# sjpark0905/DNA-LDPC-codes

Hardware: AMD Instinct MI355X
Metric: decoded codewords/sec (n=18432, m=2048, 50 BP iters) at 1/2/4/8 GPUs; % HBM roofline (higher is better)
Workload: dtype f64; 1 GPU; bsc-p0.02-100k-per-gpu-bp50; code=decode_n18432_m2048_final.pchk (8,72)-regular, E=147456, input=int8 channel codes in HBM + table code*ln49 (LR = host exp), batch_per_gpu=100000, global_batch=100000, max_iter=50, algo=bp, parallelism=dp1 (contiguous codeword shards, no collective), resident_per_pass=192, group_tiles=3, nontemporal_d=False, continuous=True, resident_pool=True, syndrome_split=False

## Files before the change

dna-ldpc-codes_amd/csrc/engine.hip:

```cpp
#include <hip/hip_ext.h>
#include <hip/hip_runtime.h>

#include <algorithm>
#include <cmath>
#include <cstdio>
#include <cstdlib>
#include <cstring>
#include <thread>

#include "engine.hpp"
#include "kernels.hpp"
#include "kernels_int.hpp"
#include "encode_kernels.hpp"

namespace ldpc {

constexpr int32_t kDefaultGroupTiles = 3;
constexpr int32_t kDefaultMsaGroupTiles = 8;
constexpr int32_t kDefaultVarCpw = 4;
constexpr int32_t kDefaultVarCpwCoded = 2;
constexpr int32_t kDefaultPoolTiles = 3;
constexpr int32_t kDefaultResPoll = 8;
constexpr int32_t kDefaultSynBlocks = 32;
constexpr int64_t kMsaPool = 1024;
constexpr int64_t kResAutoMaxTiles = 4;
constexpr int kProbes = 4;

constexpr int32_t kDefaultFlags = LDPC_SCHED_NONTEMPORAL | LDPC_SCHED_CONTINUOUS | LDPC_SCHED_MSA_COMPRESSED |
                                  LDPC_SCHED_RESIDENT | LDPC_SCHED_FIRST_FROM_PRIOR | LDPC_SCHED_LR_TABLE;
constexpr int32_t kAllFlags = kDefaultFlags | LDPC_SCHED_DEBUG_NO_DRAIN | LDPC_SCHED_DEBUG_BAD_LANE;

constexpr int32_t kResolved = 1 << 30, kResChosen = 1 << 29;

ldpc_schedule resolve_schedule(const ldpc_schedule* s)
{
    ldpc_schedule r{};
    if (s) r = *s;
    r.flags_set &= kAllFlags;
    r.flags = (kDefaultFlags & ~r.flags_set) | (r.flags & r.flags_set);
    r.flags &= kAllFlags;
    r.flags_set = kAllFlags | kResolved | ((r.flags_set & LDPC_SCHED_RESIDENT) ? kResChosen : 0);
    if (r.group_tiles == 0) r.group_tiles = -2;
    if (r.var_cpw < 1 || r.var_cpw > 8 || (r.var_cpw > 4 && r.var_cpw != 8)) r.var_cpw = -2;
    if (r.pool_tiles <= 0) r.pool_tiles = 0;
// ... 29 lines not shown
    return 2 * g.E * 8 + (int64_t)g.N * 8 + (g.N + 7) / 8 + 8;
}

Engine::~Engine()
{
    if (device >= 0) hipSetDevice(device);
    if (stream) hipStreamSynchronize(stream);
    for (int c = 0; c < K_NCLASS; c++)
        for (auto& p : ev_live[c]) { hipEventDestroy(p.first); hipEventDestroy(p.second); }
    for (auto e : ev_pool) hipEventDestroy(e);
    hipFree(d_fresh); hipFree(d_occ); hipFree(d_lane_b); hipFree(d_lane_n); hipFree(d_ctr);
    if (h_poll) hipHostFree(h_poll);
    if (h_fault) hipHostFree(h_fault);
    hipFree(d_row_ptr); hipFree(d_col_idx); hipFree(d_col_idx_T); hipFree(d_col_ptr); hipFree(d_col_edge); hipFree(d_col_er); hipFree(d_row_pos);
    hipFree(d_unsat); hipFree(d_done); hipFree(d_fin); hipFree(d_fin_b); hipFree(d_fin_n);
    hipFree(d_sgn);
    hipFree(v2c); if (c2v != v2c) hipFree(c2v); hipFree(prior); hipFree(hard); hipFree(active); hipFree(iters); hipFree(valid);
    hipFree(post_t);
    hipFree(pcode); hipFree(d_ptab); hipFree(d_expand);
    if (h_ptab) hipHostFree(h_ptab);
    if (stream) hipStreamDestroy(stream);
}

template <typename T>
static int upload(T** dst, const std::vector<T>& v)
{
    const size_t n = std::max<size_t>(v.size(), 1);
    LDPC_HIP(hipMalloc((void**)dst, n * sizeof(T)));
    if (!v.empty()) LDPC_HIP(hipMemcpy(*dst, v.data(), v.size() * sizeof(T), hipMemcpyHostToDevice));
    return LDPC_OK;
// ... 49 lines not shown

    const bool reg_72_8 = g->regular_dc && g->dc_max == 72 && g->regular_dv && g->dv_max == 8;
    msa_c = algo == LDPC_ALGO_MSA && reg_72_8 && g->N % 16 == 0 && g->E < ((int64_t)1 << dev::MSA_ER_SHIFT) &&
            sched_flag(sched, LDPC_SCHED_MSA_COMPRESSED);
    cont = sched_flag(sched, LDPC_SCHED_CONTINUOUS) && !int_algo &&
           (reg_72_8 || (g->regular_dv && g->dv_max == 8) || gen_bucket(g->dv_max, kGenVarBuckets) != 0);
    const bool gen_res = !reg_72_8 && gen_bucket(g->dc_max, kGenCheckBuckets) != 0 &&
                         gen_bucket(g->dv_max, kGenVarBuckets) != 0;
    res = sched_flag(sched, LDPC_SCHED_RESIDENT) && cont && !msa_c && ((reg_72_8 && g->N % 32 == 0) || gen_res);
    const bool res_chosen = (sched.flags_set & kResChosen) != 0;
    if (res && !res_chosen && chunk > kResAutoMaxTiles * 64) res = false;
    if (res && !res_chosen && reg_72_8 && sched.pool_tiles <= 0 &&
        64.0 * 8.0 * kDefaultPoolTiles * ((double)g->E + (double)g->N) > 1.15 * kGenPoolBytes)
        res = false;
    nt_d = sched_flag(sched, LDPC_SCHED_NONTEMPORAL) && !res;
    debug_no_drain = sched_flag(sched, LDPC_SCHED_DEBUG_NO_DRAIN);
    debug_bad_lane = sched_flag(sched, LDPC_SCHED_DEBUG_BAD_LANE);
    var_cpw = sched.var_cpw;
    res_poll = sched.poll_every;
    if (chunk <= 0) {
        size_t fr = 0, tot = 0;
        LDPC_HIP(hipMemGetInfo(&fr, &tot));
        const int64_t ptiles = sched.pool_tiles > 0 ? sched.pool_tiles : reg_72_8 ? kDefaultPoolTiles : gen_pool_tiles(*g);
        const int64_t want = res ? 64 * ptiles : (msa_c && cont) ? kMsaPool : 16384;
        chunk = std::min<int64_t>(want, (int64_t)(fr / 2) / engine_bytes_per_codeword(*g));
    }
    cap = std::max<int64_t>(64, (chunk + 63) / 64 * 64);
    cap_tiles = cap / 64;
    if (cap_tiles > 65535) { set_error("chunk too large (max 4194240 codewords)"); return LDPC_ERR_ARG; }
    int64_t group = sched.group_tiles;
// ... 35 lines not shown
        LDPC_HIP(hipMalloc((void**)&d_lane_n, (size_t)cap * sizeof(int32_t)));
        LDPC_HIP(hipMalloc((void**)&d_ctr, (size_t)(1 + kRing) * sizeof(unsigned long long)));
        LDPC_HIP(hipHostMalloc((void**)&h_poll, (size_t)kRing * sizeof(unsigned long long),
                               hipHostMallocCoherent | hipHostMallocMapped));
        std::memset(h_poll, 0, (size_t)kRing * sizeof(unsigned long long));
        LDPC_HIP(hipHostGetDevicePointer((void**)&d_poll, h_poll, 0));
        LDPC_HIP(hipHostMalloc((void**)&h_fault, dev::kFaultWords * sizeof(unsigned long long),
                               hipHostMallocCoherent | hipHostMallocMapped));
        std::memset(h_fault, 0, dev::kFaultWords * sizeof(unsigned long long));
        LDPC_HIP(hipHostGetDevicePointer((void**)&d_fault, h_fault, 0));
        LDPC_HIP(hipMalloc((void**)&d_unsat, (size_t)cap_tiles * sizeof(unsigned long long)));
        LDPC_HIP(hipMalloc((void**)&d_done, (size_t)cap_tiles * sizeof(unsigned int)));
        LDPC_HIP(hipMalloc((void**)&d_fin, (size_t)cap_tiles * sizeof(uint64_t)));
        LDPC_HIP(hipMalloc((void**)&d_fin_b, (size_t)cap * sizeof(int64_t)));
        LDPC_HIP(hipMalloc((void**)&d_fin_n, (size_t)cap * sizeof(int32_t)));
        syn_blocks = res ? 0 : sched.syn_blocks;
        first_fp = !res && reg_72_8 && algo == LDPC_ALGO_BP && sched_flag(sched, LDPC_SCHED_FIRST_FROM_PRIOR);
    }
    const size_t E = (size_t)std::max<int64_t>(g->E, 1);
    LDPC_HIP(hipMalloc((void**)&v2c, (size_t)cap * E * sizeof(double)));
    if (res) {
        c2v_tiles = cap_tiles;
        c2v = v2c;
    } else {
        c2v_tiles = std::max<int64_t>(group_tiles, cont ? (cap_tiles + 3) / 4 : 0);
        c2v_bytes = msa_c ? msa_scratch_bytes(c2v_tiles, g->M) : (size_t)c2v_tiles * 64 * E * sizeof(double);
        LDPC_HIP(hipMalloc((void**)&c2v, c2v_bytes));
    }
    LDPC_HIP(hipMalloc((void**)&prior, (size_t)cap * g->N * sizeof(double)));
    if (msa_c) LDPC_HIP(hipMalloc((void**)&d_sgn, (size_t)cap * g->N));
    LDPC_HIP(hipMalloc((void**)&hard, (size_t)cap_tiles * g->N * sizeof(uint64_t)));
    LDPC_HIP(hipMalloc((void**)&active, (size_t)cap_tiles * sizeof(uint64_t)));
    LDPC_HIP(hipMalloc((void**)&iters, (size_t)cap * sizeof(int32_t)));
    LDPC_HIP(hipMalloc((void**)&valid, (size_t)cap * sizeof(uint8_t)));
    if (!int_algo && (res || group_tiles < cap_tiles)) return probe(kProbes);
    return LDPC_OK;
}

int32_t Engine::flags() const
{
    return (nt_d ? LDPC_SCHED_NONTEMPORAL : 0) | (cont ? LDPC_SCHED_CONTINUOUS : 0) |
           (msa_c ? LDPC_SCHED_MSA_COMPRESSED : 0) | (res ? LDPC_SCHED_RESIDENT : 0) |
           (syn_blocks > 0 ? LDPC_SCHED_SPLIT_SYNDROME : 0) | (first_fp ? LDPC_SCHED_FIRST_FROM_PRIOR : 0) |
           (sched.flags & (LDPC_SCHED_LR_TABLE | LDPC_SCHED_DEBUG_NO_DRAIN | LDPC_SCHED_DEBUG_BAD_LANE));
}

int Engine::probe(int probes)
{
    const size_t E = (size_t)std::max<int64_t>(g->E, 1);
    const size_t bytes = res ? (size_t)cap * E * sizeof(double) : c2v_bytes;
    const unsigned gt = (unsigned)(res ? cap_tiles : std::min<int64_t>(group_tiles, cap_tiles));
    LDPC_HIP(hipMemsetAsync(v2c, 0, (size_t)gt * 64 * E * sizeof(double), stream));
    LDPC_HIP(hipMemsetAsync(prior, 0, (size_t)gt * 64 * g->N * sizeof(double), stream));
    LDPC_HIP(hipMemsetAsync(active, 0xff, (size_t)gt * sizeof(uint64_t), stream));
    if (d_sgn) LDPC_HIP(hipMemsetAsync(d_sgn, 0, (size_t)gt * 64 * g->N, stream));
    std::vector<double*> cand{res ? v2c : c2v};
    for (int i = 1; i < probes; i++) {
        double* p = nullptr;
// ... 632 lines not shown

int Engine::run_cont_steps(const double* d_in, int in_kind, int64_t B, int32_t max_iter, uint8_t* d_hard,
                           double* d_post, int post_kind, int32_t* d_iters, uint8_t* d_valid)
{
    using namespace dev;
    const int msa = algo == LDPC_ALGO_MSA;
    if (msa && in_kind == LDPC_IN_LR) { set_error("min-sum takes LLR input"); return LDPC_ERR_ARG; }
    if (msa && post_kind == LDPC_POST_RATIO) { set_error("LDPC_POST_RATIO is BP-only"); return LDPC_ERR_ARG; }
    if (!d_hard || !d_iters || !d_valid) { set_error("continuous mode needs hard, iters and valid outputs"); return LDPC_ERR_ARG; }
    const int32_t M = g->M, N = g->N;
    const int64_t tiles = std::min<int64_t>(cap_tiles, (B + 63) / 64);
    if (d_post && !post_t) LDPC_HIP(hipMalloc((void**)&post_t, (size_t)cap * N * sizeof(double)));
    double* pt = d_post ? post_t : nullptr;
    static_assert(1 + kRing <= 256, "occupancy ring");
    LAUNCH(K_OTHER, klaunch(k_cont_reset, dim3((unsigned)std::min<int64_t>((tiles + 255) / 256, 1024)), dim3(256), 0,
                            stream, active, d_fresh, d_occ, d_ctr, 1 + kRing, d_unsat, d_done, tiles));
    ContState cs{active, d_fresh, d_occ, d_lane_b, d_lane_n, d_ctr, nullptr, B};
    cs.ntiles = tiles;
    cs.fault = d_fault;
    cs.debug_bad_lane = debug_bad_lane ? 1 : 0;
    const uint64_t q0 = poll_seq;
    ResStep rs{hard, d_col_idx, d_unsat, d_done, d_fin, d_fin_b, d_fin_n, N, max_iter, cs, ContOut{d_iters, d_valid},
               d_row_ptr};
    const bool syn72 = g->regular_dc && g->dc_max == 72;
    const int hard_vec = ((uintptr_t)d_hard % 8 == 0 && N % 8 == 0) ? 1 : 0;
    Refill rf{d_fresh, d_lane_b, d_in, in_kind == LDPC_IN_LLR ? 1 : 0, d_fin, d_fin_b, d_fin_n,
              d_hard, d_post, post_kind == LDPC_POST_RATIO ? 1 : 0, hard_vec};
    rf.nb = B;
    rf.fault = d_fault;
    if (cur_codes) {
        rf.in = nullptr;
        rf.in_code = cur_codes;
        rf.pcode = pcode;
        rf.ptab = d_ptab;
    }
    const bool single_fill = B <= tiles * 64;
    const int lag = single_fill ? 1 : kLag;
    const int64_t lanes = tiles * 64;
    const int64_t windows = (B + lanes - 1) / lanes + 1;
    auto step_limit = [&](int64_t every) {
        return windows * ((int64_t)max_iter + 2) + (int64_t)(lag + 2) * every + 8;
    };
    auto drained = [&](unsigned long long occ) { return occ == 0 && !debug_no_drain; };
    auto overrun = [&](int64_t steps) {
// ... 165 lines not shown
```

dna-ldpc-codes_amd/csrc/engine.hpp:

```cpp
#pragma once
#include <hip/hip_runtime.h>

#include <cstdint>
#include <memory>
#include <mutex>
#include <string>
#include <vector>

#include "../../include/ldpc_amd.h"
#include "graph.hpp"
#include "kargs.hpp"

namespace ldpc {

void set_error(const std::string& msg);
const char* last_error();

#define LDPC_HIP(call)                                                                           \
    do {                                                                                         \
        hipError_t _e = (call);                                                                  \
        if (_e != hipSuccess) {                                                                  \
            ::ldpc::set_error(std::string(#call) + ": " + hipGetErrorString(_e));                \
            return LDPC_ERR_DEVICE;                                                              \
        }                                                                                        \
// ... 8 lines not shown
    const HostGraph* g = nullptr;
    int device = 0;
    int algo = LDPC_ALGO_BP;
    hipStream_t stream = nullptr;
    ldpc_schedule sched{};
    int64_t cap = 0;
    int64_t cap_tiles = 0;
    int64_t group_tiles = 0;
    int64_t c2v_tiles = 0;
    size_t c2v_bytes = 0;
    bool nt_d = false;
    bool cont = false;
    bool msa_c = false;
    bool res = false;
    bool first_fp = false;
    bool debug_no_drain = false;
    bool debug_bad_lane = false;
    int var_cpw = 4;
    int res_poll = 8;
    int syn_blocks = 0;
    uint8_t* d_sgn = nullptr;
    unsigned long long* d_unsat = nullptr;
    unsigned int* d_done = nullptr;
    uint64_t* d_fin = nullptr;
    int64_t* d_fin_b = nullptr;
    int32_t* d_fin_n = nullptr;
    const dev::ResStep* rstep = nullptr;
    static constexpr int kRing = 8, kLag = 2;
    uint64_t* d_fresh = nullptr;
    uint64_t* d_occ = nullptr;
    int64_t* d_lane_b = nullptr;
    int32_t* d_lane_n = nullptr;
    unsigned long long* d_ctr = nullptr;
    uint64_t poll_seq = 0;
    unsigned long long* h_poll = nullptr;
    unsigned long long* d_poll = nullptr;
    void poll_arm(dev::ContState& cs, uint64_t q) const;
    int poll_wait(uint64_t q, unsigned long long* occ);
    unsigned long long* h_fault = nullptr;
    unsigned long long* d_fault = nullptr;
    int check_fault();
// ... 89 lines not shown
```

dna-ldpc-codes_amd/csrc/kargs.hpp:

```cpp
#pragma once
#include <cstdint>

namespace ldpc {
namespace dev {

struct Refill {
    const uint64_t* fresh;
    const int64_t* lane_b;
    const double* in;
    int in_is_llr;
    const uint64_t* fin;
    const int64_t* fin_b;
    const int32_t* fin_n;
    uint8_t* hard_out;
    double* post_out;
    int post_ratio;
    int hard_vec;
    int prior_only = 0;
    const int8_t* in_code = nullptr;
    int8_t* pcode = nullptr;
    const double* ptab = nullptr;
    int64_t nb = 0;
    unsigned long long* fault = nullptr;
};

constexpr unsigned long long kFaultTag = 1ull << 63;
constexpr unsigned long long kFaultIndex = (1ull << 48) - 1ull;
enum FaultKind : unsigned {
    kFaultIters = 1,
    kFaultOutput = 2,
    kFaultRefill = 3,
    kFaultSchedule = 4
};
constexpr int kFaultWords = 5;

constexpr int kCodeBias = 128;

struct ContState {
// ... 20 lines not shown
    uint8_t* valid;
};

struct ResStep {
    const uint64_t* hard;
    const int32_t* col_idx;
    unsigned long long* unsat;
    unsigned int* done;
    uint64_t* fin;
    int64_t* fin_b;
    int32_t* fin_n;
    int32_t N, max_iter;
    ContState cs;
    ContOut co;
    const int32_t* row_ptr = nullptr;
};

}
}
```

dna-ldpc-codes_amd/csrc/kernels.hpp:

```cpp
#pragma once
#include <hip/hip_runtime.h>
#include <cstdint>

#include "kargs.hpp"

namespace ldpc {
namespace dev {

constexpr int TILE = 64;

__device__ __forceinline__ int wave_id() { return __builtin_amdgcn_readfirstlane((int)(threadIdx.x >> 6)); }
__device__ __forceinline__ int lane_id() { return (int)(threadIdx.x & 63); }

__device__ __forceinline__ unsigned xcd_block(unsigned b, unsigned nb)
{
    const unsigned q = nb / 8, r = nb % 8, x = b % 8;
    return (x < r ? x * (q + 1) : r * (q + 1) + (x - r) * q) + b / 8;
}

__device__ __forceinline__ uint64_t shfl_xor_u64(uint64_t v, int m)
{
    uint32_t lo = (uint32_t)v, hi = (uint32_t)(v >> 32);
    lo = (uint32_t)__shfl_xor((int)lo, m);
    hi = (uint32_t)__shfl_xor((int)hi, m);
// ... 68 lines not shown
#pragma unroll
        for (int c = 0; c < CPW; ++c) p[c] = (uint8_t)(v >> (8 * c));
    }
}

__host__ __device__ __forceinline__ uint64_t splitmix64(uint64_t x)
{
    x += 0x9E3779B97F4A7C15ull;
    x = (x ^ (x >> 30)) * 0xBF58476D1CE4E5B9ull;
    x = (x ^ (x >> 27)) * 0x94D049BB133111EBull;
    return x ^ (x >> 31);
}

__device__ __forceinline__ void cont_lanes(int64_t t, uint64_t occ, uint64_t U, int32_t max_iter, const ContState& cs,
                                           const ContOut& co, int64_t* s_b, int32_t* s_n, uint64_t* s_fin,
                                           int32_t ln0, int64_t b0, bool probe)
{
    const int lane = lane_id();
    {
        const size_t li = (size_t)t * TILE + lane;
        const bool o = (occ >> lane) & 1ull;
        const int32_t ln = o ? ln0 : 0;
        const bool unsat = (U >> lane) & 1ull;
        const bool fin = o && (!unsat || ln == max_iter);
        const bool cont = o && !fin;
        const int64_t b = o ? b0 : -1;
        if (fin && lane_index_ok(b, cs.B, cs.fault, kFaultIters)) { co.iters[b] = ln; co.valid[b] = unsat ? 0 : 1; }
        s_b[lane] = b;
        s_n[lane] = ln;
        const uint64_t F = __ballot(fin), Cm = __ballot(cont);
        const uint64_t freem = ~Cm;
        const int nfree = __popcll(freem);
        unsigned long long base = 0;
        if (lane == 0 && nfree > 0) {
            if (probe) {
                const unsigned long long nb = __hip_atomic_load(cs.next_b, __ATOMIC_RELAXED, __HIP_MEMORY_SCOPE_AGENT);
                base = (nb < (unsigned long long)cs.B) ? atomicAdd(cs.next_b, (unsigned long long)nfree) : nb;
            } else {
                base = atomicAdd(cs.next_b, (unsigned long long)nfree);
            }
        }
        base = __shfl(base, 0);
        const int rank = __popcll(freem & ((1ull << lane) - 1ull));
        const bool fresh = !cont && (base + (unsigned long long)rank < (unsigned long long)cs.B);
        const uint64_t Fr = __ballot(fresh);
        if (cont) cs.lane_n[li] = ln + 1;
        if (fresh) {
            int64_t nbv = (int64_t)(base + rank);
            if (cs.debug_bad_lane && nbv == 0) nbv = cs.B + 4096;
            cs.lane_b[li] = nbv;
            cs.lane_n[li] = 0;
        }
        if (lane == 0) {
            cs.active[t] = Cm;
            cs.fresh[t] = Fr;
            cs.occupied[t] = Cm | Fr;
            *s_fin = F;
            if (cs.occ_count) {
                const unsigned long long add = (1ull << kOccTileShift) | (unsigned long long)__popcll(Cm | Fr);
                const unsigned long long old = atomicAdd(cs.occ_count, add);
                if (cs.poll_host && (int64_t)(old >> kOccTileShift) + 1 == cs.ntiles)
                    __hip_atomic_store(cs.poll_host, (cs.poll_tag << kOccTileShift) | ((old + add) & kOccMask),
                                       __ATOMIC_RELAXED, __HIP_MEMORY_SCOPE_SYSTEM);
            }
            if (t == 0 && cs.occ_clear) *cs.occ_clear = 0ull;
        }
    }
}

template <int DC>
__device__ __forceinline__ uint64_t row_parity(const uint64_t* __restrict__ h, const int32_t* __restrict__ cols)
{
    const int lane = lane_id();
    uint64_t p = 0;
#pragma unroll
    for (int k0 = 0; k0 < DC; k0 += TILE)
        if (k0 + lane < DC) p ^= h[cols[k0 + lane]];
#pragma unroll
    for (int off = 32; off > 0; off >>= 1) p ^= shfl_xor_u64(p, off);
    return p;
}

__device__ __forceinline__ void res_arrive(int64_t t, uint64_t occ, uint64_t p, const ResStep& rs, int32_t ln0,
                                           int64_t b0, uint32_t nblk)
{
    __shared__ uint64_t red[4];
    __shared__ int64_t s_b[TILE];
    __shared__ int32_t s_n[TILE];
    __shared__ uint64_t s_fin;
    __shared__ int s_last;
    const int lane = lane_id(), w = wave_id();
    if (lane == 0) red[w] = p;
    __syncthreads();
    if (threadIdx.x == 0) {
        const uint64_t U = red[0] | red[1] | red[2] | red[3];
        unsigned long long o = 0;
        if (U) o = atomicOr(rs.unsat + t, (unsigned long long)U);
        asm volatile("" ::"v"(o) : "memory");
        s_last = atomicAdd(rs.done + t, 1u) == nblk - 1;
    }
    __syncthreads();
    if (!s_last) return;
    if (threadIdx.x < TILE) {
        const uint64_t U = occ ? (uint64_t)atomicOr(rs.unsat + t, 0ull) : 0ull;
        cont_lanes(t, occ, U, rs.max_iter, rs.cs, rs.co, s_b, s_n, &s_fin, ln0, b0, false);
        const size_t li = (size_t)t * TILE + lane;
        rs.fin_b[li] = s_b[lane];
        rs.fin_n[li] = s_n[lane];
        if (lane == 0) {
            rs.fin[t] = s_fin;
            atomicExch(rs.unsat + t, 0ull);
            atomicExch(rs.done + t, 0u);
        }
    }
}

__global__ __launch_bounds__(256) void k_init(const double* __restrict__ in, int in_is_llr, int algo_msa,
                                              int64_t Bc, int32_t N, int64_t E,
                                              const int32_t* __restrict__ col_ptr, const int32_t* __restrict__ col_edge,
                                              double* __restrict__ prior, double* __restrict__ v2c,
                                              uint64_t* __restrict__ hard, uint64_t* __restrict__ active,
                                              int32_t* __restrict__ iters, uint8_t* __restrict__ valid,
                                              uint8_t* __restrict__ sgn, int32_t vpa, int32_t vpb)
{
    __shared__ double s[TILE][TILE + 1];
    const int lane = lane_id(), w = wave_id();
// ... 130 lines not shown
    const int lane = lane_id();
    const int32_t row = (int32_t)rb * 4 + wave_id();
    const uint64_t act = RES ? rs.cs.occupied[t] : active[t];
    const auto src = dmsg + ((size_t)t * E + (size_t)row * DC) * TILE + lane;
    const auto dst = lr_t + (size_t)row * DC * TILE + lane;
    if constexpr (!RES) {
        if (!(row < M && line_occupied(act, lane))) return;
        double x[DC];
        check_bp_load<DC, NT, false>(x, src);
        check_bp_compute<DC, false>(x, dst);
    } else {
        static_assert(DC <= 2 * TILE, "row parity: two gathers per lane");
        const bool occ_l = (act >> lane) & 1ull;
        const int32_t ln0 = rs.cs.lane_n[t * TILE + lane];
        const int64_t b0 = rs.cs.lane_b[t * TILE + lane];
        uint64_t par = 0;
        if (row < M && act != 0) {
            const int32_t* __restrict__ cols = rs.col_idx + (size_t)row * DC;
            const int32_t c0 = cols[lane < DC ? lane : DC - 1];
            const int32_t c1 = cols[TILE + lane < DC ? TILE + lane : DC - 1];
            double x[DC];
            check_bp_load<DC, NT, true>(x, src);
            int32_t d0 = c0, d1 = c1;
            asm volatile("" : "+v"(d0), "+v"(d1));
            const uint64_t* __restrict__ h = rs.hard + (size_t)t * rs.N;
            const uint64_t g0 = h[d0];
            const uint64_t g1 = h[d1];
            check_bp_compute<DC, true>(x, dst);
            uint64_t p = (lane < DC ? g0 : 0ull) ^ (TILE + lane < DC ? g1 : 0ull);
#pragma unroll
            for (int off = 32; off > 0; off >>= 1) p ^= shfl_xor_u64(p, off);
            par = p;
        }
        res_arrive(t, act, par, rs, occ_l ? ln0 : 0, occ_l ? b0 : 0, nrb);
    }
}

template <int DC, bool PC = false>
__global__ __launch_bounds__(256, 2) void k_check_bp_first(const double* __restrict__ prior,
                                                           const int8_t* __restrict__ pcode,
                                                           const double* __restrict__ ptab,
                                                           const int32_t* __restrict__ col_idx,
                                                           double* __restrict__ lr, const uint64_t* __restrict__ active,
                                                           int32_t M, int32_t N, int64_t E, int64_t t0)
{
    const int lane = lane_id();
    const int32_t row = (int32_t)blockIdx.x * 4 + wave_id();
    const int64_t t = t0 + blockIdx.y;
    const uint64_t act = active[t];
// ... 101 lines not shown

template <bool MSA, int DV, bool NT, bool CONT, int CPW, bool INPLACE, bool PC = false>
__device__ __forceinline__ void var_m_block(typename Msg<INPLACE>::in c2v_t, typename Msg<INPLACE>::out v2c,
                                            double* __restrict__ prior, uint64_t* __restrict__ hard,
                                            const uint64_t* __restrict__ active, const int32_t* __restrict__ col_edge,
                                            double* __restrict__ post, int32_t N, int64_t E, int64_t t, uint32_t cb,
                                            const Refill& rf)
{
    const int lane = lane_id();
    const int32_t j0 = ((int32_t)cb * 4 + wave_id()) * CPW;
    if (j0 >= N) return;
    const uint64_t act = active[t];
    const uint64_t frm = CONT ? rf.fresh[t] : 0ull;
    const uint64_t touched = act | frm;
    const uint64_t fm = (CONT && rf.fin) ? rf.fin[t] : 0ull;
    if (touched == 0 && fm == 0) return;
    const bool live = (act >> lane) & 1ull;
    const bool fr = CONT && ((frm >> lane) & 1ull);
    const bool fl = (fm >> lane) & 1ull;
    int64_t fb = 0;
    int32_t fn = 0;
    if (fl) {
        fb = rf.fin_b[t * TILE + lane];
        fn = rf.fin_n[t * TILE + lane];
    }
    const size_t tb = (size_t)t * E;
    int32_t eid[CPW][DV];
#pragma unroll
    for (int c = 0; c < CPW; ++c)
#pragma unroll
        for (int s = 0; s < DV; ++s) eid[c][s] = col_edge[(size_t)(j0 + c) * DV + s];
    double l[CPW][DV], pv[CPW], xin[CPW];
    int8_t kin[CPW];
    bool bad_in = false;
// ... 8 lines not shown
        }
    }
    if (live) {
#pragma unroll
        for (int c = 0; c < CPW; ++c) {
            pv[c] = prior_at<PC>(prior, rf, ((size_t)t * N + j0 + c) * TILE + lane);
#pragma unroll
            for (int s = 0; s < DV; ++s) l[c][s] = c2v_t[(size_t)eid[c][s] * TILE + lane];
        }
    }
    if constexpr (PC) {
        if (fr) {
#pragma unroll
            for (int c = 0; c < CPW; ++c) xin[c] = rf.ptab[kin[c] + kCodeBias];
        }
    }
    const bool fok = out_ok(fb, rf);
    if (CONT && fl && fok) {
        uint64_t hw[CPW];
#pragma unroll
        for (int c = 0; c < CPW; ++c) hw[c] = hard[(size_t)t * N + j0 + c];
        store_fin_hard<CPW>(rf, hw, fb, N, j0, lane);
    }
#pragma unroll
    for (int c = 0; c < CPW; ++c) {
        const int32_t j = j0 + c;
        const size_t pj = ((size_t)t * N + j) * TILE + lane;
        if (CONT && fl && fok && rf.post_out) {
            const size_t ob = (size_t)fb * N + j;
            const double pv = fn > 0 ? post[pj] : prior_at<PC>(prior, rf, pj);
// ... 12 lines not shown
        if (fr) {
            const double x = xin[c];
            if (MSA) {
                np = x;
#pragma unroll
                for (int s = 0; s < DV; ++s) dv[s] = x;
                h = !(x > 0);
            } else {
                const double LR0 = (!PC && rf.in_is_llr) ? exp(x) : x;
                np = LR0;
                const double d0 = 1.0 - 2.0 / (1.0 + LR0);
#pragma unroll
                for (int s = 0; s < DV; ++s) dv[s] = d0;
                h = (LR0 < 1.0);
            }
        } else if (live) {
            if (MSA) {
#pragma unroll
                for (int s = 0; s < DV; ++s) {
                    double sum = pv[c];
#pragma unroll
                    for (int r = 0; r < DV; ++r)
                        if (r != s) sum = sum + l[c][r];
                    dv[s] = sum;
                }
                double L = pv[c];
#pragma unroll
                for (int s = 0; s < DV; ++s) L = L + l[c][s];
                h = !(L > 0);
                if (post) post[pj] = L;
            } else {
// ... 133 lines not shown
__global__ __launch_bounds__(256) void k_check_msa(typename Msg<RES>::in v2c, typename Msg<RES>::out c2v,
                                                   const uint64_t* __restrict__ active, int32_t M, int64_t E,
                                                   int64_t t0, ResStep rs)
{
    const int lane = lane_id();
    const int32_t row = blockIdx.x * 4 + wave_id();
    const int64_t t = t0 + blockIdx.y;
    const uint64_t act = RES ? rs.cs.occupied[t] : active[t];
    const bool run = row < M && line_occupied(act, lane);
    if constexpr (!RES) {
        if (!run) return;
    }
    uint64_t par = 0;
    int32_t ln0 = 0;
    int64_t b0 = 0;
    if (RES && act != 0) {
        if (threadIdx.x < TILE && ((act >> lane) & 1ull)) {
            ln0 = rs.cs.lane_n[t * TILE + lane];
            b0 = rs.cs.lane_b[t * TILE + lane];
        }
        if (row < M) par = row_parity<DC>(rs.hard + (size_t)t * rs.N, rs.col_idx + (size_t)row * DC);
    }
    if (run)
        check_msa_row<DC, NT, RES>(v2c + ((size_t)t * E + (size_t)row * DC) * TILE + lane,
                                   c2v + ((size_t)blockIdx.y * E + (size_t)row * DC) * TILE + lane);
    if constexpr (RES) res_arrive(t, act, par, rs, ln0, b0, gridDim.x);
}

__global__ __launch_bounds__(256) void k_check_msa_gen(const double* __restrict__ v2c, double* __restrict__ c2v,
                                                       const uint64_t* __restrict__ active,
                                                       const int32_t* __restrict__ row_ptr, int32_t M, int64_t E,
                                                       int64_t t0)
{
    const int lane = lane_id();
    const int32_t row = blockIdx.x * 4 + wave_id();
    const int64_t t = t0 + blockIdx.y;
    if (row >= M) return;
    const uint64_t act = active[t];
    if (!((act >> lane) & 1ull)) return;
    const int32_t a = row_ptr[row], b = row_ptr[row + 1];
    const size_t tb = (size_t)t * E, tl = (size_t)blockIdx.y * E;
// ... 773 lines not shown
    const size_t pj = ((size_t)t * N + j) * TILE + lane;
    double out;
    if (algo_msa) {
        out = iters[b] > 0 ? post_t[pj] : prior[pj];
    } else {
        double P = iters[b] > 0 ? post_t[pj] : prior[pj];
        if (__builtin_isnan(P)) P = 1.0;
        out = post_ratio ? P : log(P);
    }
    post[(size_t)b * N + j] = out;
}

__global__ __launch_bounds__(256) void k_cont_reset(uint64_t* __restrict__ active, uint64_t* __restrict__ fresh,
                                                    uint64_t* __restrict__ occupied, unsigned long long* __restrict__ ctr,
                                                    int32_t nctr, unsigned long long* __restrict__ unsat,
                                                    unsigned* __restrict__ done, int64_t tiles)
{
    for (int64_t i = (int64_t)blockIdx.x * blockDim.x + threadIdx.x; i < tiles; i += (int64_t)gridDim.x * blockDim.x) {
        active[i] = 0;
        fresh[i] = 0;
        occupied[i] = 0;
        if (unsat) unsat[i] = 0;
        if (done) done[i] = 0;
    }
    if (blockIdx.x == 0 && (int32_t)threadIdx.x < nctr) ctr[threadIdx.x] = 0;
}

template <int DC>
__global__ __launch_bounds__(256) void k_syndrome_split(int32_t M, ResStep rs, uint32_t tiles)
{
    constexpr int KP = (DC + 7) / 8;
    const int64_t t = blockIdx.x % tiles;
    const uint32_t blk = blockIdx.x / tiles, nblk = gridDim.x / tiles;
    const uint64_t occ = rs.cs.occupied[t];
    const int lane = lane_id();
    int32_t ln0 = 0;
    int64_t b0 = 0;
    uint64_t u = 0;
// ... 123 lines not shown
```

dna-ldpc-codes_amd/ldpc_amd.py:

```python
from __future__ import annotations

import ctypes as C
import enum
import math
import os
import threading
import time
from typing import Optional, Sequence

import numpy as np

_HERE = os.path.dirname(os.path.abspath(__file__))
LIB_PATH = os.path.join(_HERE, "lib", "libldpc_amd.so")

ABI_VERSION = 3
LDPC_OK, LDPC_ERR_ARG, LDPC_ERR_IO, LDPC_ERR_FORMAT, LDPC_ERR_DEVICE, LDPC_ERR_UNSUPPORTED = 0, -1, -2, -3, -4, -5


class Algo(enum.IntEnum):
    BP = 0
    MSA = 1
    QMSA = 2
    GALLAGER_A = 3
    GALLAGER_B1 = 4
# ... 9 lines not shown
_NAMES = {"bp": ALGO_BP, "msa": ALGO_MSA, "min-sum": ALGO_MSA, "qmsa": ALGO_QMSA,
          "gallager_a": ALGO_GALLAGER_A, "gallager_b1": ALGO_GALLAGER_B1, "gallager_b2": ALGO_GALLAGER_B2}
DECODER_TYPES = {0: ALGO_BP, 1: ALGO_GALLAGER_A, 2: ALGO_GALLAGER_B1, 3: ALGO_GALLAGER_B2,
                 20: ALGO_MSA, 21: ALGO_MSA, 22: ALGO_MSA}
_RESULT_TYPE = {ALGO_BP: 0, ALGO_GALLAGER_A: 1, ALGO_GALLAGER_B1: 2, ALGO_GALLAGER_B2: 3, ALGO_MSA: 20,
                ALGO_QMSA: 21}


class LdpcError(RuntimeError):
    def __init__(self, code: int, msg: str):
        super().__init__(f"ldpc_amd error {code}: {msg}")
        self.code = code


SCHED_FLAGS = {"nontemporal": 1 << 0, "continuous": 1 << 3, "msa_compressed": 1 << 4, "resident": 1 << 5,
               "split_syndrome": 1 << 6, "first_from_prior": 1 << 12, "lr_table": 1 << 13,
               "debug_no_drain": 1 << 14, "debug_bad_lane": 1 << 15}
SCHED_FIELDS = ("group_tiles", "var_cpw", "pool_tiles", "poll_every", "syn_blocks")


class Schedule(C.Structure):
    _fields_ = [("flags_set", C.c_int32), ("flags", C.c_int32), ("group_tiles", C.c_int32), ("var_cpw", C.c_int32),
                ("pool_tiles", C.c_int32), ("poll_every", C.c_int32), ("syn_blocks", C.c_int32),
                ("reserved", C.c_int32)]

    @classmethod
    def make(cls, **kw) -> "Schedule":
        s = cls()
        for k, v in kw.items():
            if v is None:
                continue
# ... 450 lines not shown
        sch = Schedule.make(**kw)
        err = C.c_int(0)
        self._h = lib().ldpc_engine_create_ex(g.handle, device, self.algo, chunk, C.byref(sch), C.byref(err))
        if not self._h:
            raise LdpcError(err.value, (lib().ldpc_last_error() or b"").decode())
        cap, grp, fl = C.c_int64(), C.c_int64(), C.c_int32()
        _check(lib().ldpc_engine_info(self._h, C.byref(cap), C.byref(grp), C.byref(fl)))
        self.cap, self.group_tiles, self.flags = cap.value, grp.value, fl.value
        f = fl.value
        self.nontemporal = bool(f & SCHED_FLAGS["nontemporal"])
        self.continuous = bool(f & SCHED_FLAGS["continuous"])
        self.msa_compressed = bool(f & SCHED_FLAGS["msa_compressed"])
        self.resident = bool(f & SCHED_FLAGS["resident"])
        self.syndrome_split = bool(f & SCHED_FLAGS["split_syndrome"])
        self.first_from_prior = bool(f & SCHED_FLAGS["first_from_prior"])

    def decode(self, d_in, in_kind: int, B: int, max_iter: int, d_hard=None, d_post=None, post_kind=POST_LLR,
               d_iters=None, d_valid=None):
        _check(lib().ldpc_engine_decode(self._h, d_in, in_kind, B, max_iter, d_hard, d_post, post_kind, d_iters,
                                        d_valid))

    def decode_codes(self, d_codes, table: np.ndarray, table_kind: int, B: int, max_iter: int, d_hard=None,
                     d_post=None, post_kind=POST_LLR, d_iters=None, d_valid=None):
        t = np.ascontiguousarray(table, dtype=np.float64)
        if t.shape != (256,):
            raise ValueError("the code table has 256 entries (code + 128)")
        _check(lib().ldpc_engine_decode_codes(self._h, d_codes, _ptr(t), table_kind, B, max_iter, d_hard, d_post,
                                              post_kind, d_iters, d_valid))

    def set_params(self, msa_precision: int = 6, msa_step: float = 0.5, msa_offset: int = 0, tie_seed: int = 0):
# ... 102 lines not shown
```

include/ldpc_amd.h:

```cpp
#ifndef LDPC_AMD_H
#define LDPC_AMD_H

#include <stddef.h>
#include <stdint.h>

#ifdef __cplusplus
extern "C" {
#endif

#define LDPC_AMD_ABI_VERSION 3

enum {
    LDPC_OK = 0,
    LDPC_ERR_ARG = -1,
    LDPC_ERR_IO = -2,
    LDPC_ERR_FORMAT = -3,
    LDPC_ERR_DEVICE = -4,
    LDPC_ERR_UNSUPPORTED = -5
};

enum {
    LDPC_ALGO_BP = 0,
    LDPC_ALGO_MSA = 1,
    LDPC_ALGO_QMSA = 2,
// ... 8 lines not shown
};

enum {
    LDPC_IN_LLR = 0,
    LDPC_IN_LR = 1
};

typedef struct ldpc_graph ldpc_graph;

enum {
    LDPC_SCHED_NONTEMPORAL = 1 << 0,
    LDPC_SCHED_CONTINUOUS = 1 << 3,
    LDPC_SCHED_MSA_COMPRESSED = 1 << 4,
    LDPC_SCHED_RESIDENT = 1 << 5,
    LDPC_SCHED_SPLIT_SYNDROME = 1 << 6,
    LDPC_SCHED_FIRST_FROM_PRIOR = 1 << 12,
    LDPC_SCHED_LR_TABLE = 1 << 13,
    LDPC_SCHED_DEBUG_NO_DRAIN = 1 << 14,
    LDPC_SCHED_DEBUG_BAD_LANE = 1 << 15
};

typedef struct ldpc_schedule {
    int32_t flags_set;
    int32_t flags;
    int32_t group_tiles;
    int32_t var_cpw;
    int32_t pool_tiles;
    int32_t poll_every;
    int32_t syn_blocks;
    int32_t reserved;
// ... 177 lines not shown
```

Before: 27410 codewords/s.

## Hand over final-iteration lanes early so fresh codewords start during last pass

Adds a default-on handover schedule for the resident BP/MSA path. Lanes about to run their final iteration are freed and refilled with new codewords in the same step. The pending codeword's final hard decision and posterior are written out by the variable kernel, and its syndrome is checked a step later from a separate hard_fin buffer. This aims to cut lane idle time in the last iteration of the continuous pipeline. In exchange it adds extra per-tile state, a second parity reduction per row, and a hard_fin buffer sized tiles×N.

```diff
diff --git a/dna-ldpc-codes_amd/csrc/engine.hip b/dna-ldpc-codes_amd/csrc/engine.hip
--- a/dna-ldpc-codes_amd/csrc/engine.hip
+++ b/dna-ldpc-codes_amd/csrc/engine.hip
@@ -27,7 +27,8 @@
 constexpr int kProbes = 4;
 
 constexpr int32_t kDefaultFlags = LDPC_SCHED_NONTEMPORAL | LDPC_SCHED_CONTINUOUS | LDPC_SCHED_MSA_COMPRESSED |
-                                  LDPC_SCHED_RESIDENT | LDPC_SCHED_FIRST_FROM_PRIOR | LDPC_SCHED_LR_TABLE;
+                                  LDPC_SCHED_RESIDENT | LDPC_SCHED_FIRST_FROM_PRIOR | LDPC_SCHED_LR_TABLE |
+                                  LDPC_SCHED_HANDOVER;
 constexpr int32_t kAllFlags = kDefaultFlags | LDPC_SCHED_DEBUG_NO_DRAIN | LDPC_SCHED_DEBUG_BAD_LANE;
 
 constexpr int32_t kResolved = 1 << 30, kResChosen = 1 << 29;
@@ -87,6 +88,7 @@
     if (h_fault) hipHostFree(h_fault);
     hipFree(d_row_ptr); hipFree(d_col_idx); hipFree(d_col_idx_T); hipFree(d_col_ptr); hipFree(d_col_edge); hipFree(d_col_er); hipFree(d_row_pos);
     hipFree(d_unsat); hipFree(d_done); hipFree(d_fin); hipFree(d_fin_b); hipFree(d_fin_n);
+    hipFree(d_ho); hipFree(d_pend_b); hipFree(hard_fin);
     hipFree(d_sgn);
     hipFree(v2c); if (c2v != v2c) hipFree(c2v); hipFree(prior); hipFree(hard); hipFree(active); hipFree(iters); hipFree(valid);
     hipFree(post_t);
@@ -166,6 +168,8 @@
         64.0 * 8.0 * kDefaultPoolTiles * ((double)g->E + (double)g->N) > 1.15 * kGenPoolBytes)
         res = false;
     nt_d = sched_flag(sched, LDPC_SCHED_NONTEMPORAL) && !res;
+    handover = sched_flag(sched, LDPC_SCHED_HANDOVER) && res && reg_72_8 &&
+               (algo == LDPC_ALGO_BP || algo == LDPC_ALGO_MSA);
     debug_no_drain = sched_flag(sched, LDPC_SCHED_DEBUG_NO_DRAIN);
     debug_bad_lane = sched_flag(sched, LDPC_SCHED_DEBUG_BAD_LANE);
     var_cpw = sched.var_cpw;
@@ -231,6 +235,11 @@
         LDPC_HIP(hipMalloc((void**)&d_fin, (size_t)cap_tiles * sizeof(uint64_t)));
         LDPC_HIP(hipMalloc((void**)&d_fin_b, (size_t)cap * sizeof(int64_t)));
         LDPC_HIP(hipMalloc((void**)&d_fin_n, (size_t)cap * sizeof(int32_t)));
+        if (handover) {
+            LDPC_HIP(hipMalloc((void**)&d_ho, (size_t)cap_tiles * 3 * sizeof(uint64_t)));
+            LDPC_HIP(hipMalloc((void**)&d_pend_b, (size_t)cap * sizeof(int64_t)));
+            LDPC_HIP(hipMalloc((void**)&hard_fin, (size_t)cap_tiles * g->N * sizeof(uint64_t)));
+        }
         syn_blocks = res ? 0 : sched.syn_blocks;
         first_fp = !res && reg_72_8 && algo == LDPC_ALGO_BP && sched_flag(sched, LDPC_SCHED_FIRST_FROM_PRIOR);
     }
@@ -259,6 +268,7 @@
     return (nt_d ? LDPC_SCHED_NONTEMPORAL : 0) | (cont ? LDPC_SCHED_CONTINUOUS : 0) |
            (msa_c ? LDPC_SCHED_MSA_COMPRESSED : 0) | (res ? LDPC_SCHED_RESIDENT : 0) |
            (syn_blocks > 0 ? LDPC_SCHED_SPLIT_SYNDROME : 0) | (first_fp ? LDPC_SCHED_FIRST_FROM_PRIOR : 0) |
+           (handover ? LDPC_SCHED_HANDOVER : 0) |
            (sched.flags & (LDPC_SCHED_LR_TABLE | LDPC_SCHED_DEBUG_NO_DRAIN | LDPC_SCHED_DEBUG_BAD_LANE));
 }
 
@@ -921,7 +931,7 @@
     double* pt = d_post ? post_t : nullptr;
     static_assert(1 + kRing <= 256, "occupancy ring");
     LAUNCH(K_OTHER, klaunch(k_cont_reset, dim3((unsigned)std::min<int64_t>((tiles + 255) / 256, 1024)), dim3(256), 0,
-                            stream, active, d_fresh, d_occ, d_ctr, 1 + kRing, d_unsat, d_done, tiles));
+                            stream, active, d_fresh, d_occ, d_ctr, 1 + kRing, d_unsat, d_done, tiles, d_ho, cap_tiles));
     ContState cs{active, d_fresh, d_occ, d_lane_b, d_lane_n, d_ctr, nullptr, B};
     cs.ntiles = tiles;
     cs.fault = d_fault;
@@ -935,6 +945,16 @@
               d_hard, d_post, post_kind == LDPC_POST_RATIO ? 1 : 0, hard_vec};
     rf.nb = B;
     rf.fault = d_fault;
+    if (handover) {
+        rs.last = d_ho;
+        rs.pend = d_ho + cap_tiles;
+        rs.unsat_fin = reinterpret_cast<unsigned long long*>(d_ho + 2 * cap_tiles);
+        rs.pend_b = d_pend_b;
+        rs.hard_fin = hard_fin;
+        rf.last = rs.last;
+        rf.pend_b = d_pend_b;
+        rf.hard_fin = hard_fin;
+    }
     if (cur_codes) {
         rf.in = nullptr;
         rf.in_code = cur_codes;
diff --git a/dna-ldpc-codes_amd/csrc/engine.hpp b/dna-ldpc-codes_amd/csrc/engine.hpp
--- a/dna-ldpc-codes_amd/csrc/engine.hpp
+++ b/dna-ldpc-codes_amd/csrc/engine.hpp
@@ -46,6 +46,7 @@
     bool msa_c = false;
     bool res = false;
     bool first_fp = false;
+    bool handover = false;
     bool debug_no_drain = false;
     bool debug_bad_lane = false;
     int var_cpw = 4;
@@ -57,6 +58,9 @@
     uint64_t* d_fin = nullptr;
     int64_t* d_fin_b = nullptr;
     int32_t* d_fin_n = nullptr;
+    uint64_t* d_ho = nullptr;
+    int64_t* d_pend_b = nullptr;
+    uint64_t* hard_fin = nullptr;
     const dev::ResStep* rstep = nullptr;
     static constexpr int kRing = 8, kLag = 2;
     uint64_t* d_fresh = nullptr;
diff --git a/dna-ldpc-codes_amd/csrc/kargs.hpp b/dna-ldpc-codes_amd/csrc/kargs.hpp
--- a/dna-ldpc-codes_amd/csrc/kargs.hpp
+++ b/dna-ldpc-codes_amd/csrc/kargs.hpp
@@ -22,6 +22,9 @@
     const double* ptab = nullptr;
     int64_t nb = 0;
     unsigned long long* fault = nullptr;
+    const uint64_t* last = nullptr;
+    const int64_t* pend_b = nullptr;
+    uint64_t* hard_fin = nullptr;
 };
 
 constexpr unsigned long long kFaultTag = 1ull << 63;
@@ -72,6 +75,11 @@
     ContState cs;
     ContOut co;
     const int32_t* row_ptr = nullptr;
+    uint64_t* last = nullptr;
+    uint64_t* pend = nullptr;
+    int64_t* pend_b = nullptr;
+    const uint64_t* hard_fin = nullptr;
+    unsigned long long* unsat_fin = nullptr;
 };
 
 }
diff --git a/dna-ldpc-codes_amd/csrc/kernels.hpp b/dna-ldpc-codes_amd/csrc/kernels.hpp
--- a/dna-ldpc-codes_amd/csrc/kernels.hpp
+++ b/dna-ldpc-codes_amd/csrc/kernels.hpp
@@ -106,11 +106,19 @@
 
 __device__ __forceinline__ void cont_lanes(int64_t t, uint64_t occ, uint64_t U, int32_t max_iter, const ContState& cs,
                                            const ContOut& co, int64_t* s_b, int32_t* s_n, uint64_t* s_fin,
-                                           int32_t ln0, int64_t b0, bool probe)
+                                           int32_t ln0, int64_t b0, bool probe, const ResStep* ho = nullptr,
+                                           uint64_t pend = 0, uint64_t Up = 0)
 {
     const int lane = lane_id();
     {
         const size_t li = (size_t)t * TILE + lane;
+        if (ho && ((pend >> lane) & 1ull)) {
+            const int64_t pb = ho->pend_b[li];
+            if (lane_index_ok(pb, cs.B, cs.fault, kFaultIters)) {
+                co.iters[pb] = max_iter;
+                co.valid[pb] = ((Up >> lane) & 1ull) ? 0 : 1;
+            }
+        }
         const bool o = (occ >> lane) & 1ull;
         const int32_t ln = o ? ln0 : 0;
         const bool unsat = (U >> lane) & 1ull;
@@ -120,8 +128,9 @@
         if (fin && lane_index_ok(b, cs.B, cs.fault, kFaultIters)) { co.iters[b] = ln; co.valid[b] = unsat ? 0 : 1; }
         s_b[lane] = b;
         s_n[lane] = ln;
-        const uint64_t F = __ballot(fin), Cm = __ballot(cont);
-        const uint64_t freem = ~Cm;
+        const bool last = ho && cont && ln + 1 == max_iter;
+        const uint64_t F = __ballot(fin), Cm = __ballot(cont), Lm = __ballot(last);
+        const uint64_t freem = ~Cm | Lm;
         const int nfree = __popcll(freem);
         unsigned long long base = 0;
         if (lane == 0 && nfree > 0) {
@@ -134,9 +143,10 @@
         }
         base = __shfl(base, 0);
         const int rank = __popcll(freem & ((1ull << lane) - 1ull));
-        const bool fresh = !cont && (base + (unsigned long long)rank < (unsigned long long)cs.B);
+        const bool fresh = (!cont || last) && (base + (unsigned long long)rank < (unsigned long long)cs.B);
         const uint64_t Fr = __ballot(fresh);
         if (cont) cs.lane_n[li] = ln + 1;
+        if (last) ho->pend_b[li] = b;
         if (fresh) {
             int64_t nbv = (int64_t)(base + rank);
             if (cs.debug_bad_lane && nbv == 0) nbv = cs.B + 4096;
@@ -146,7 +156,8 @@
         if (lane == 0) {
             cs.active[t] = Cm;
             cs.fresh[t] = Fr;
-            cs.occupied[t] = Cm | Fr;
+            cs.occupied[t] = (Cm & ~Lm) | Fr;
+            if (ho) { ho->last[t] = Lm; ho->pend[t] = Lm; }
             *s_fin = F;
             if (cs.occ_count) {
                 const unsigned long long add = (1ull << kOccTileShift) | (unsigned long long)__popcll(Cm | Fr);
@@ -173,21 +184,36 @@
     return p;
 }
 
+__device__ __forceinline__ uint64_t pend_lanes(const ResStep& rs, int64_t t) { return rs.pend ? rs.pend[t] : 0ull; }
+template <int DC>
+__device__ __forceinline__ uint64_t pend_parity(const ResStep& rs, int64_t t, int32_t row, int32_t M, uint64_t pend)
+{
+    if (pend == 0 || row >= M) return 0ull;
+    return row_parity<DC>(rs.hard_fin + (size_t)t * rs.N, rs.col_idx + (size_t)row * DC) & pend;
+}
+
 __device__ __forceinline__ void res_arrive(int64_t t, uint64_t occ, uint64_t p, const ResStep& rs, int32_t ln0,
-                                           int64_t b0, uint32_t nblk)
-{
-    __shared__ uint64_t red[4];
+                                           int64_t b0, uint32_t nblk, uint64_t pend = 0, uint64_t pp = 0)
+{
+    __shared__ uint64_t red[4], redp[4];
     __shared__ int64_t s_b[TILE];
     __shared__ int32_t s_n[TILE];
     __shared__ uint64_t s_fin;
     __shared__ int s_last;
     const int lane = lane_id(), w = wave_id();
-    if (lane == 0) red[w] = p;
+    if (lane == 0) {
+        red[w] = p;
+        redp[w] = pp;
+    }
     __syncthreads();
     if (threadIdx.x == 0) {
         const uint64_t U = red[0] | red[1] | red[2] | red[3];
         unsigned long long o = 0;
         if (U) o = atomicOr(rs.unsat + t, (unsigned long long)U);
+        if (pend) {
+            const uint64_t Up = redp[0] | redp[1] | redp[2] | redp[3];
+            if (Up) o |= atomicOr(rs.unsat_fin + t, (unsigned long long)Up);
+        }
         asm volatile("" ::"v"(o) : "memory");
         s_last = atomicAdd(rs.done + t, 1u) == nblk - 1;
     }
@@ -195,13 +221,16 @@
     if (!s_last) return;
     if (threadIdx.x < TILE) {
         const uint64_t U = occ ? (uint64_t)atomicOr(rs.unsat + t, 0ull) : 0ull;
-        cont_lanes(t, occ, U, rs.max_iter, rs.cs, rs.co, s_b, s_n, &s_fin, ln0, b0, false);
+        const uint64_t Up = pend ? (uint64_t)atomicOr(rs.unsat_fin + t, 0ull) : 0ull;
+        cont_lanes(t, occ, U, rs.max_iter, rs.cs, rs.co, s_b, s_n, &s_fin, ln0, b0, false, rs.last ? &rs : nullptr, pend,
+                   Up);
         const size_t li = (size_t)t * TILE + lane;
         rs.fin_b[li] = s_b[lane];
         rs.fin_n[li] = s_n[lane];
         if (lane == 0) {
             rs.fin[t] = s_fin;
             atomicExch(rs.unsat + t, 0ull);
+            if (pend) atomicExch(rs.unsat_fin + t, 0ull);
             atomicExch(rs.done + t, 0u);
         }
     }
@@ -362,6 +391,7 @@
         const bool occ_l = (act >> lane) & 1ull;
         const int32_t ln0 = rs.cs.lane_n[t * TILE + lane];
         const int64_t b0 = rs.cs.lane_b[t * TILE + lane];
+        const uint64_t pend = pend_lanes(rs, t);
         uint64_t par = 0;
         if (row < M && act != 0) {
             const int32_t* __restrict__ cols = rs.col_idx + (size_t)row * DC;
@@ -380,7 +410,7 @@
             for (int off = 32; off > 0; off >>= 1) p ^= shfl_xor_u64(p, off);
             par = p;
         }
-        res_arrive(t, act, par, rs, occ_l ? ln0 : 0, occ_l ? b0 : 0, nrb);
+        res_arrive(t, act, par, rs, occ_l ? ln0 : 0, occ_l ? b0 : 0, nrb, pend, pend_parity<DC>(rs, t, row, M, pend));
     }
 }
 
@@ -512,10 +542,13 @@
     const uint64_t frm = CONT ? rf.fresh[t] : 0ull;
     const uint64_t touched = act | frm;
     const uint64_t fm = (CONT && rf.fin) ? rf.fin[t] : 0ull;
+    constexpr bool HO = CONT && INPLACE;
+    const uint64_t lastm = (HO && rf.last) ? rf.last[t] : 0ull;
     if (touched == 0 && fm == 0) return;
     const bool live = (act >> lane) & 1ull;
     const bool fr = CONT && ((frm >> lane) & 1ull);
     const bool fl = (fm >> lane) & 1ull;
+    const bool ls = HO && ((lastm >> lane) & 1ull);
     int64_t fb = 0;
     int32_t fn = 0;
     if (fl) {
@@ -554,6 +587,34 @@
 #pragma unroll
             for (int c = 0; c < CPW; ++c) xin[c] = rf.ptab[kin[c] + kCodeBias];
         }
+    }
+    if (HO && lastm != 0) {
+        const int64_t lb = ls ? rf.pend_b[t * TILE + lane] : 0;
+        const bool lok = out_ok(lb, rf);
+        uint64_t hwf[CPW];
+#pragma unroll
+        for (int c = 0; c < CPW; ++c) {
+            bool hf = false;
+            if (ls) {
+                double p = pv[c];
+                if (MSA) {
+#pragma unroll
+                    for (int s = 0; s < DV; ++s) p = p + l[c][s];
+                    hf = !(p > 0);
+                    if (lok && rf.post_out) rf.post_out[(size_t)lb * N + j0 + c] = p;
+                } else {
+#pragma unroll
+                    for (int s = 0; s < DV; ++s) p = p * l[c][s];
+                    if (__builtin_isnan(p)) p = 1.0;
+                    hf = (p <= 1.0);
+                    if (lok && rf.post_out) rf.post_out[(size_t)lb * N + j0 + c] = rf.post_ratio ? p : log(p);
+                }
+            }
+            hwf[c] = __ballot(hf);
+            if (lane == 0) rf.hard_fin[(size_t)t * N + j0 + c] = hwf[c];
+        }
+        if (ls && lok) store_fin_hard<CPW>(rf, hwf, lb, N, j0, lane);
+        if (ls && !lok) lane_fault(rf.fault, kFaultOutput, t * TILE + lane);
     }
     const bool fok = out_ok(fb, rf);
     if (CONT && fl && fok) {
@@ -596,7 +657,7 @@
                 for (int s = 0; s < DV; ++s) dv[s] = d0;
                 h = (LR0 < 1.0);
             }
-        } else if (live) {
+        } else if (live && !ls) {
             if (MSA) {
 #pragma unroll
                 for (int s = 0; s < DV; ++s) {
@@ -760,17 +821,19 @@
     uint64_t par = 0;
     int32_t ln0 = 0;
     int64_t b0 = 0;
+    const uint64_t pend = RES ? pend_lanes(rs, t) : 0ull;
     if (RES && act != 0) {
         if (threadIdx.x < TILE && ((act >> lane) & 1ull)) {
             ln0 = rs.cs.lane_n[t * TILE + lane];
             b0 = rs.cs.lane_b[t * TILE + lane];
         }
         if (row < M) par = row_parity<DC>(rs.hard + (size_t)t * rs.N, rs.col_idx + (size_t)row * DC);
-    }
-    if (run)
+    }    if (run)
         check_msa_row<DC, NT, RES>(v2c + ((size_t)t * E + (size_t)row * DC) * TILE + lane,
                                    c2v + ((size_t)blockIdx.y * E + (size_t)row * DC) * TILE + lane);
-    if constexpr (RES) res_arrive(t, act, par, rs, ln0, b0, gridDim.x);
+    if constexpr (RES) {
+        res_arrive(t, act, par, rs, ln0, b0, gridDim.x, pend, pend_parity<DC>(rs, t, row, M, pend));
+    }
 }
 
 __global__ __launch_bounds__(256) void k_check_msa_gen(const double* __restrict__ v2c, double* __restrict__ c2v,
@@ -1574,7 +1637,8 @@
 __global__ __launch_bounds__(256) void k_cont_reset(uint64_t* __restrict__ active, uint64_t* __restrict__ fresh,
                                                     uint64_t* __restrict__ occupied, unsigned long long* __restrict__ ctr,
                                                     int32_t nctr, unsigned long long* __restrict__ unsat,
-                                                    unsigned* __restrict__ done, int64_t tiles)
+                                                    unsigned* __restrict__ done, int64_t tiles,
+                                                    uint64_t* __restrict__ ho, int64_t ho_stride)
 {
     for (int64_t i = (int64_t)blockIdx.x * blockDim.x + threadIdx.x; i < tiles; i += (int64_t)gridDim.x * blockDim.x) {
         active[i] = 0;
@@ -1582,6 +1646,11 @@
         occupied[i] = 0;
         if (unsat) unsat[i] = 0;
         if (done) done[i] = 0;
+        if (ho) {
+            ho[i] = 0;
+            ho[ho_stride + i] = 0;
+            ho[2 * ho_stride + i] = 0;
+        }
     }
     if (blockIdx.x == 0 && (int32_t)threadIdx.x < nctr) ctr[threadIdx.x] = 0;
 }
diff --git a/dna-ldpc-codes_amd/ldpc_amd.py b/dna-ldpc-codes_amd/ldpc_amd.py
--- a/dna-ldpc-codes_amd/ldpc_amd.py
+++ b/dna-ldpc-codes_amd/ldpc_amd.py
@@ -47,7 +47,7 @@
 
 
 SCHED_FLAGS = {"nontemporal": 1 << 0, "continuous": 1 << 3, "msa_compressed": 1 << 4, "resident": 1 << 5,
-               "split_syndrome": 1 << 6, "first_from_prior": 1 << 12, "lr_table": 1 << 13,
+               "split_syndrome": 1 << 6, "handover": 1 << 7, "first_from_prior": 1 << 12, "lr_table": 1 << 13,
                "debug_no_drain": 1 << 14, "debug_bad_lane": 1 << 15}
 SCHED_FIELDS = ("group_tiles", "var_cpw", "pool_tiles", "poll_every", "syn_blocks")
 
@@ -528,6 +528,7 @@
         self.resident = bool(f & SCHED_FLAGS["resident"])
         self.syndrome_split = bool(f & SCHED_FLAGS["split_syndrome"])
         self.first_from_prior = bool(f & SCHED_FLAGS["first_from_prior"])
+        self.handover = bool(f & SCHED_FLAGS["handover"])
 
     def decode(self, d_in, in_kind: int, B: int, max_iter: int, d_hard=None, d_post=None, post_kind=POST_LLR,
                d_iters=None, d_valid=None):
diff --git a/include/ldpc_amd.h b/include/ldpc_amd.h
--- a/include/ldpc_amd.h
+++ b/include/ldpc_amd.h
@@ -46,6 +46,7 @@
     LDPC_SCHED_MSA_COMPRESSED = 1 << 4,
     LDPC_SCHED_RESIDENT = 1 << 5,
     LDPC_SCHED_SPLIT_SYNDROME = 1 << 6,
+    LDPC_SCHED_HANDOVER = 1 << 7,
     LDPC_SCHED_FIRST_FROM_PRIOR = 1 << 12,
     LDPC_SCHED_LR_TABLE = 1 << 13,
     LDPC_SCHED_DEBUG_NO_DRAIN = 1 << 14,
```

Result: faster. 27750 codewords/s (median of 6 runs) (+1.2%).
